# DrawZeroPoint/Structure-Light-Reconstructor

Hardware: AMD Instinct MI355X
Metric: Mpixels/s decode+unwrap+triangulate, 4096x3000 stereo, 1/2/4/8 GPU (higher is better)
Workload: dtype u8 in, f32 phase/XYZ (f64 undistort + Q reprojection)

## Files before the change

structure-light-reconstructor_amd/capi.py:

```python
import ctypes as C
import os

import numpy as np

_HERE = os.path.dirname(os.path.abspath(__file__))
LIB_PATH = os.path.join(_HERE, "libslr_hip.so")

MF_PLANES = 14
MAX_GRAY_BITS = 16
MEM_HOST, MEM_DEVICE = 0, 1
OPT_MF_MATCH_ALGO = 1
OPT_RECT_DECODE_ALGO = 3
OPT_RECT_DMA_SHAPE = 6
OPT_RECT_DMA_DEPTH = 7
OPT_DEBUG_RECT_RESIDENT = 8
OPT_DEBUG_FLAGS = 9
OPT_DEBUG_K4_STOP = 10
OPT_BATCH_STREAMS = 12
OPT_DEBUG_POISON_SCRATCH = 13
OPT_MF_BATCH_GROUP = 15
OPT_MF_BATCH_DECODE_GROUP = 16
OPT_EVAL_MODEL = 14
OPT_HYBRID_ONE_PASS = 11
OPT_PROFILE_STRIDE = 5
# ... 39 lines not shown
    _fields_ = [("W", C.c_int), ("H", C.c_int), ("mf_form", C.c_int), ("dma_shape", C.c_int), ("dma_depth", C.c_int),
                ("dma_tiles", C.c_uint), ("dma_nofit_tiles", C.c_uint), ("quads_by_class", C.c_uint * 3),
                ("waves_by_mode", C.c_uint * 3), ("lds_nofit_tiles", C.c_uint * 2), ("dma_extra_entries", C.c_uint)]


class FuseDesc(C.Structure):
    _fields_ = [("n_frames", C.c_int), ("W", C.c_int), ("H", C.c_int), ("voxel", C.c_double), ("origin", C.c_double * 3),
                ("min_points", C.c_uint32), ("max_voxels", C.c_uint32)]


class FuseStats(C.Structure):
    _fields_ = [("points", C.c_uint64), ("distinct", C.c_uint64), ("table_entries", C.c_uint64), ("atomics", C.c_uint64)]


DEBUG_FUSE_COUNT_ATOMICS = 512

MODE_GRAY, MODE_GE, MODE_MF = 0, 1, 2
ASSIGN_CYCLIC, ASSIGN_BLOCKED = 0, 1


class Calib(C.Structure):
    _fields_ = [("cam", Camera * 2), ("Q", C.c_double * 16), ("T", C.c_float * 12), ("has_T", C.c_int)]


def make_camera(fc, cc, k, R=None, t=None):
    cam = Camera()
    cam.fc[:] = [float(v) for v in fc]
    cam.cc[:] = [float(v) for v in cc]
    kk = list(k) + [0.0] * (5 - len(k))
    cam.k[:] = [float(v) for v in kk]
# ... 724 lines not shown
```

structure-light-reconstructor_amd/csrc/kernels_rectdma.hip:

```cpp
#include "decode_common.hpp"

#include <stdlib.h>

#if !defined(SLR_EXPERIMENTS) && (defined(SLR_DMA_ABL) || defined(SLR_DMA_FORCE_MODE) || defined(SLR_DMA_CLOCKPROBE))
#error "SLR_DMA_ABL / SLR_DMA_FORCE_MODE / SLR_DMA_CLOCKPROBE are experiment switches: build with -DSLR_EXPERIMENTS"
#endif

namespace slr {

constexpr unsigned kDmaInvalid = 0x80000000u;

template <int TW, int TH, int NT>
struct DmaGeom {
    static constexpr int NWAVES = NT / 64;
    static constexpr int PX = TW * TH / NT;
    static constexpr int NQ = PX / 4;
    static constexpr int QPR = TW / 4;
    static constexpr int BR = TH >= 8 ? 8 : TH, BC = 64 / BR;
    static_assert(QPR % BC == 0 && TH % BR == 0, "quad blocks");
    static __device__ __host__ constexpr int quad_row(int g) { return (g / 64) / (QPR / BC) * BR + (g % 64) / BC; }
    static __device__ __host__ constexpr int quad_col(int g) { return ((g / 64) % (QPR / BC) * BC + (g % 64) % BC) * 4; }
    static constexpr int WPR = TW / 64;
    static constexpr int RPP = NWAVES / WPR;
    static constexpr int CMAX = TW / 16 + 2;
// ... 297 lines not shown
}

struct DmaJob {
    const uint8_t *base;
    unsigned pstride;
    unsigned fringe_skip;
    unsigned stack_bytes;
    const int4 *boxes;
    const unsigned *digest;
    unsigned digest_bytes;
    unsigned entries;
    float *phase;
    uint8_t *valid;
};
struct DmaJobs { DmaJob j[kDmaMaxJobs]; };

__device__ __forceinline__ void dma16(unsigned voff, __amdgpu_buffer_rsrc_t rsrc, unsigned lds_dst, unsigned soff)
{
    unsigned keep;
    asm volatile("s_mov_b32 %0, m0\n\ts_mov_b32 m0, %3\n\ts_nop 0\n\tbuffer_load_dwordx4 %1, %2, %4 offen lds\n\ts_mov_b32 m0, %0"
                 : "=&s"(keep) : "v"(voff), "s"(rsrc), "s"(__builtin_amdgcn_readfirstlane(lds_dst)), "s"(__builtin_amdgcn_readfirstlane(soff)) : "memory");
}

template <int N>
__device__ __forceinline__ void wait_vm()
{
    static_assert(N >= 0 && N < 64, "vmcnt is a 6-bit counter");
    asm volatile("s_waitcnt vmcnt(%0)" :: "n"(N) : "memory");
}

// ... 162 lines not shown
        }
    } else {
        DmaRd r[2];
        dma_rd<IMG0, IMG1, RS>(r[0], tap[0].a0);
#pragma unroll
        for (int q = 0; q < PX; q++) {
            if (q + 1 < PX) { dma_rd<IMG0, IMG1, RS>(r[(q + 1) & 1], tap[q + 1].a0); dma_rd_wait<8>(r[q & 1]); }
            else dma_rd_wait<0>(r[q & 1]);
            sd[q] = (int)(dma_blend(r[q & 1], 0, tap[q]) >> 16) - (int)(dma_blend(r[q & 1], 1, tap[q]) >> 16);
        }
    }
}

constexpr int kDmaDigestPhase = 3;
template <int PX, int A, int PLANE_DMAS = 2>
__device__ __host__ constexpr int dma_wait_count(int p)
{
    int n = 0;
    for (int j = 1; j < A; j++) { const int ph = ((p - A + j) % 7 + 7) % 7; n += PLANE_DMAS + (ph == kDmaDigestPhase ? PX / 4 : 0); }
    return n;
}

constexpr int kSubBands = 4;
struct DmaPool {
    int pb;
    int per;
    int T, E;
    int per_x;
    __device__ __host__ static DmaPool of(int T, int E = 0, int x = 0)
    {
        DmaPool p;
        p.pb = (T + 8 * kSubBands - 1) / (8 * kSubBands); p.per = kSubBands * p.pb; p.T = T; p.E = E > T ? E : T;
        p.per_x = 0;
        for (int k = 0; k < kSubBands; k++) {
// ... 99 lines not shown
        if (!has_next) { voff_next = kDmaInvalid; nxt_act = false; }
    }
};

template <int TW, int TH, int NT, int A, bool HASVALID, bool X87 = false>
struct DmaDecode {
    typedef DmaGeom<TW, TH, NT> Gm;
    static constexpr int PX = Gm::PX, PS = Gm::PS, RS = Gm::RS, D = A + 1;
    static constexpr bool SPLIT = 2 * Gm::NCH <= NT;
    static constexpr int PLANE_DMAS = SPLIT ? 1 : 2;
    static constexpr int DIG_OFF = D * 2 * PS, DIG_BYTES = TW * TH * 4;
    static constexpr int WT_OFF = DIG_OFF + DIG_BYTES, WT1_OFF = WT_OFF + 1026 * 4, WT_BYTES = 2 * 1026 * 4;
    static constexpr int TAP_WT = WT_OFF;
    static constexpr int LUT_OFF = WT_OFF + WT_BYTES;
    static constexpr int TKT_OFF = LUT_OFF + (kLutWords + 1) * 4;
    static constexpr int LDS_BYTES = TKT_OFF + 12;
    static_assert(WT_OFF <= 65536 && LDS_BYTES <= 160 * 1024, "DMA destinations are 16-bit LDS addresses (M0)");
    static constexpr int kSentinel = kDmaSentinel;

    const uint8_t *smem;
    const float *lut;
    unsigned lds0, wave_off;
    unsigned pslot_off;
    unsigned plane_g;
    bool plane_wave;
    __amdgpu_buffer_rsrc_t rs_stack, rs_dig, rs_phase, rs_valid;
    unsigned pstride, fringe_skip;
    int W, H, black_thr;
    DmaSched sc;
    DmaTap tap[PX];
    unsigned qbase[PX / 4];
    unsigned oslot[PX / 4];
    unsigned second;
    int mode;
    unsigned ok;
    int pm[PX];
    int dd[PX];
    int Pk[PX];
    float F12[PX];
    float outv[PX];
    unsigned out_ok;
    int out_ty, out_tx;
    bool out_pending;

// ... 34 lines not shown
                dma16(voff, rs_stack, lds0 + (unsigned)((buf * 2 + g) * PS) + pslot_off,
                      (unsigned)dma_phase_plane(p, g) * pstride + (p == 0 ? 0u : fringe_skip));
        }
    }
    __device__ __forceinline__ void issue_digest(unsigned tile, bool live) const
    {
#if defined(SLR_DMA_ABL) && (SLR_DMA_ABL == 8 || SLR_DMA_ABL == 9)
        tile = (tile & 63u) * 94u;
#endif
#pragma unroll
        for (int r = 0; r < PX / 4; r++) {
            const unsigned voff = live ? tile * (unsigned)DIG_BYTES + (threadIdx.x + (unsigned)(NT * r)) * 16u : kDmaInvalid;
            dma16(voff, rs_dig, lds0 + (unsigned)(DIG_OFF + r * NT * 16) + wave_off, 0u);
        }
    }

    static __device__ __forceinline__ float pair_q24(int Pa, int Pb) { return dma_pair_q24(Pa, Pb); }
    static __device__ __forceinline__ float finish_q24(float Fa, float Fb)
    {
        if constexpr (X87) return het_finish_x87(Fa, Fb);
        else return dma_finish_q24(Fa, Fb);
    }

    template <int K0, int P>
    __device__ __forceinline__ void phase(int ty, int tx, unsigned voff_cur)
    {
        static_assert(7 - A > 2 && kDmaDigestPhase > 2 && kDmaDigestPhase < 7, "the next tile is known from phase 2 on");
        if (plane_wave) wait_vm<dma_wait_count<PX, A, PLANE_DMAS>(P)>();
        else if (P == 0) wait_vm<0>();
#if !defined(SLR_DMA_ABL) || SLR_DMA_ABL != 3
        asm volatile("s_barrier" ::: "memory");
#endif
        if (P == 1) sc.draw();
        if constexpr (P == 2) sc.pick_up();
        if (P == kDmaDigestPhase) issue_digest((unsigned)sc.nxt, sc.has_next);
        issue_planes((P + A) % 7, (K0 + P + A) % D, P + A >= 7 ? sc.voff_next : voff_cur);
        if constexpr (P == 0) {
            if (out_pending) flush();
            const unsigned *dg = reinterpret_cast<const unsigned *>(smem + DIG_OFF + threadIdx.x * (PX * 4));
            mode = dma_tap_setup<PX, RS, TAP_WT, WT1_OFF>(smem, lds0, dg, tap, qbase, second, oslot);
            ok = 0;
        }
        constexpr unsigned img0 = (unsigned)(((K0 + P) % D) * 2 * PS), img1 = img0 + PS;
        int sd[PX];
#if defined(SLR_DMA_ABL) && (SLR_DMA_ABL == 2 || SLR_DMA_ABL == 6)
#pragma unroll
        for (int q = 0; q < PX; q++) {
            DmaRd r;
#pragma unroll
            for (int i = 0; i < 8; i++) r.v[i] = tap[q].a0 * (unsigned)(i + 3 + P);
            sd[q] = (int)(dma_blend(r, 0, tap[q]) >> 16) - (int)(dma_blend(r, 1, tap[q]) >> 16);
        }
#elif defined(SLR_DMA_ABL) && SLR_DMA_ABL == 4
#pragma unroll
        for (int q = 0; q < PX; q++) sd[q] = (int)tap[q].a0 + P;
#elif defined(SLR_DMA_ABL) && SLR_DMA_ABL == 5
        DmaRd r[2];
        dma_rd<img0, img1, (unsigned)RS>(r[0], tap[0].a0);
#pragma unroll
        for (int q = 0; q < PX; q++) {
            if (q + 1 < PX) { dma_rd<img0, img1, (unsigned)RS>(r[(q + 1) & 1], tap[q + 1].a0); dma_rd_wait<8>(r[q & 1]); }
            else dma_rd_wait<0>(r[q & 1]);
            sd[q] = (int)(r[q & 1].v[0] ^ r[q & 1].v[1] ^ r[q & 1].v[2] ^ r[q & 1].v[3] ^ r[q & 1].v[4] ^ r[q & 1].v[5] ^ r[q & 1].v[6] ^ r[q & 1].v[7]) & 255;
        }
#else
        __builtin_amdgcn_s_setprio(1);
        if constexpr (P >= 2 && (P & 1) == 0) dma_differences<PX, img1, img0, (unsigned)RS>(mode, tap, qbase, second, sd);
        else dma_differences<PX, img0, img1, (unsigned)RS>(mode, tap, qbase, second, sd);
        __builtin_amdgcn_s_setprio(0);
#endif
        if (P == 1) sc.publish();
        if constexpr (P == 0) {
#pragma unroll
            for (int q = 0; q < PX; q++) {
                if constexpr (HASVALID) ok |= (sd[q] > black_thr ? 0x10001u : 0u) << q;
                else pm[q] = sd[q] > black_thr ? (int)0x80000000 : kSentinel;
            }
        } else if constexpr ((P & 1) != 0) {
#pragma unroll
            for (int q = 0; q < PX; q++) dd[q] = sd[q];
        } else {
#pragma unroll
            for (int q = 0; q < PX; q++) {
                int nz;
                const int Pw = wrapped_nd_q24(sd[q], dd[q], lut, nz);
                if constexpr (HASVALID) { if (nz == 0) ok &= ~(1u << q); }
// ... 4 lines not shown
                    if constexpr (HASVALID) {
                        outv[q] = ((ok >> (q + 16)) & 1u) ? ph : 0.0f;
                    } else {
                        const int m3 = pm[q] > Pw ? pm[q] : Pw;
                        outv[q] = m3 != kSentinel ? ph : kInvalidPhase;
                    }
                }
            }
            if constexpr (P == 6) { out_ok = ok; out_ty = ty; out_tx = tx; out_pending = true; }
        }
    }

    template <int K0, int P>
    __device__ __forceinline__ void idle_phase(unsigned voff_cur)
    {
        if (plane_wave) wait_vm<dma_wait_count<PX, A, PLANE_DMAS>(P)>();
        else if (P == 0) wait_vm<0>();
        asm volatile("s_barrier" ::: "memory");
        if (P == 1) sc.draw();
        if constexpr (P == 2) sc.pick_up();
        if (P == kDmaDigestPhase) issue_digest((unsigned)sc.nxt, sc.has_next);
        issue_planes((P + A) % 7, (K0 + P + A) % D, P + A >= 7 ? sc.voff_next : voff_cur);
        if constexpr (P == 0) { if (out_pending) flush(); out_pending = false; }
        if (P == 1) sc.publish();
    }

    template <int K0>
    __device__ __forceinline__ void tile(int ty, int tx, bool act, unsigned voff_cur)
    {
        if (act) {
            phase<K0, 0>(ty, tx, voff_cur);
            phase<K0, 1>(ty, tx, voff_cur);
            phase<K0, 2>(ty, tx, voff_cur);
            phase<K0, 3>(ty, tx, voff_cur);
            phase<K0, 4>(ty, tx, voff_cur);
            phase<K0, 5>(ty, tx, voff_cur);
            phase<K0, 6>(ty, tx, voff_cur);
        } else {
            idle_phase<K0, 0>(voff_cur);
// ... 8 lines not shown
};

template <int LDS_BYTES, int NT>
constexpr int dma_waves_per_simd()
{
    constexpr int wgs = 160 * 1024 / LDS_BYTES, w = wgs * NT / 256;
    return w > 8 ? 8 : w < 1 ? 1 : w;
}

template <int LDS_BYTES, int NT>
constexpr int mf_dma_waves() { return dma_waves_per_simd<LDS_BYTES, NT>() > 6 ? 6 : dma_waves_per_simd<LDS_BYTES, NT>(); }

template <int TW, int TH, int NT, int A, bool HASVALID, bool X87 = false>
__global__ __launch_bounds__(NT, (HASVALID ? 4 : mf_dma_waves<DmaDecode<TW, TH, NT, A, HASVALID>::LDS_BYTES, NT>())) SLR_TICKET_KERNEL
void mf_rect_decode_dma_kernel(DmaJobs jobs, int njobs, int pitch, int W, int H, int black_thr, const float *__restrict__ lut_g,
                               int tiles_x, int tiles_y, unsigned *__restrict__ sched)
{
    typedef DmaDecode<TW, TH, NT, A, HASVALID, X87> Dec;
    typedef DmaGeom<TW, TH, NT> Gm;
    extern __shared__ __attribute__((aligned(16))) uint8_t smem[];
    Dec d;
    d.smem = smem;
    d.lds0 = __builtin_amdgcn_readfirstlane((unsigned)(uintptr_t)smem);
    if (d.lds0 & 0x1FFFu) __builtin_trap();
#if defined(SLR_DMA_CLOCKPROBE)
    const unsigned long long probe_entry = wall_clock64();
#endif
    float *lut = reinterpret_cast<float *>(smem + Dec::LUT_OFF);
    d.lut = lut;
    for (int i = threadIdx.x; i < kLutWords; i += NT) lut[i] = lut_g[i];
    if constexpr (Dec::WT_BYTES > 0)
    for (unsigned i = threadIdx.x; i < 1025u; i += NT) {
        unsigned w0, w1;
        dma_weights(i, w0, w1);
        *reinterpret_cast<unsigned *>(smem + Dec::WT_OFF + 4u * i) = w0;
        *reinterpret_cast<unsigned *>(smem + Dec::WT1_OFF + 4u * i) = w1;
    }
    __syncthreads();
    if (!HASVALID && threadIdx.x == 0)
        reinterpret_cast<int *>(lut)[kLutP + (9 << 8)] = Dec::kSentinel;
    __syncthreads();
    const unsigned nblk = gridDim.x / (unsigned)njobs;
    const int xcd = (int)(blockIdx.x & 7u), nbx = (int)(nblk >> 3);
    const int ji = (int)((blockIdx.x >> 3) % (unsigned)njobs), lb = (int)((blockIdx.x >> 3) / (unsigned)njobs);
    const int T = tiles_x * tiles_y;
    d.sc.pool = DmaPool::of(T, (int)jobs.j[ji].entries, xcd);
    int cur = d.sc.pool.entry(xcd, lb);
    if (cur < 0) {
        if (threadIdx.x == 0) dma_sched_leave(sched);
        return;
    }

    d.wave_off = __builtin_amdgcn_readfirstlane((threadIdx.x >> 6) * 1024u);
    {
        const unsigned wv = __builtin_amdgcn_readfirstlane(threadIdx.x >> 6);
        constexpr unsigned wpp = (unsigned)Gm::NCH / 64u;
        d.plane_g = Dec::SPLIT ? wv / wpp : 0u;
        d.pslot_off = (Dec::SPLIT ? wv % wpp : wv) * 1024u;
        d.plane_wave = Dec::SPLIT ? wv < 2u * wpp : wv < wpp;
    }
    d.W = W; d.H = H; d.black_thr = black_thr;
    d.sc.pitch = pitch; d.sc.W = W; d.sc.H = H;
    const int chunk = Dec::SPLIT ? (int)threadIdx.x % Gm::NCH : (int)threadIdx.x;
    d.sc.crow = chunk / Gm::CMAX; d.sc.ccol = chunk - d.sc.crow * Gm::CMAX;
    d.sc.chunk_live = Dec::SPLIT || chunk < Gm::NCH;
    d.sc.xcd = xcd; d.sc.first_ticket = nbx;
    d.sc.wave0 = __builtin_amdgcn_readfirstlane(threadIdx.x >> 6) == 0u;
    d.sc.wave_bit = 1u << __builtin_amdgcn_readfirstlane(threadIdx.x >> 6);
    d.sc.tkt_lds = d.lds0 + (unsigned)Dec::TKT_OFF;

#if defined(SLR_DMA_CLOCKPROBE)
    const unsigned long long probe_c0 = clock64(), probe_w0 = wall_clock64();
#endif
    d.pstride = jobs.j[ji].pstride; d.fringe_skip = jobs.j[ji].fringe_skip;
    d.rs_stack = __builtin_amdgcn_make_buffer_rsrc((void *)jobs.j[ji].base, 0, (int)jobs.j[ji].stack_bytes, 0x00020000);
    d.rs_dig = __builtin_amdgcn_make_buffer_rsrc((void *)jobs.j[ji].digest, 0, (int)jobs.j[ji].digest_bytes, 0x00020000);
    d.rs_phase = __builtin_amdgcn_make_buffer_rsrc((void *)jobs.j[ji].phase, 0, (int)((unsigned)W * (unsigned)H * 4u), 0x00020000);
    d.rs_valid = __builtin_amdgcn_make_buffer_rsrc((void *)jobs.j[ji].valid, 0, HASVALID ? (int)((unsigned)W * (unsigned)H) : 0, 0x00020000);
    d.sc.boxes = jobs.j[ji].boxes;
    d.sc.ctr = sched + (ji * 8 + xcd) * kSchedStride;
    d.sc.nxt = 0; d.sc.has_next = false; d.sc.voff_next = kDmaInvalid; d.sc.nxt_ty = d.sc.nxt_tx = 0; d.sc.nxt_act = false;
#if defined(SLR_DMA_CLOCKPROBE)
    int it = 0;
#define SLR_DMA_COUNT(x) ((x)++)
#else
#define SLR_DMA_COUNT(x) ((void)0)
#endif
    int cur_ty, cur_tx;
    bool cur_act;
    unsigned voff_cur = d.sc.box_voff(cur, cur_ty, cur_tx, cur_act);
    d.out_pending = false;
    d.ok = 0;
    d.issue_digest((unsigned)cur, true);
#pragma unroll
    for (int a = 0; a < A; a++) d.issue_planes(a, a % Dec::D, voff_cur);

    for (;;) {
#define SLR_DMA_TILE(K0)                                                                                       \
        {                                                                                                      \
            d.template tile<K0>(cur_ty, cur_tx, cur_act, voff_cur);                                            \
            SLR_DMA_COUNT(it);                                                                                 \
            if (!d.sc.has_next) break;                                                                         \
            cur = d.sc.nxt; voff_cur = d.sc.voff_next;                                                         \
            cur_ty = d.sc.nxt_ty; cur_tx = d.sc.nxt_tx; cur_act = d.sc.nxt_act;                                \
        }
        SLR_DMA_TILE(0)
        SLR_DMA_TILE(7 % Dec::D)
        if constexpr (Dec::D >= 3) SLR_DMA_TILE(14 % Dec::D)
        if constexpr (Dec::D >= 4) SLR_DMA_TILE(21 % Dec::D)
#undef SLR_DMA_TILE
    }
#undef SLR_DMA_COUNT
    if (d.out_pending) d.flush();
    wait_vm<0>();
    if (threadIdx.x == 0) dma_sched_leave(sched);
#if defined(SLR_DMA_CLOCKPROBE)
    if (threadIdx.x == 0) {
        unsigned long long *o = reinterpret_cast<unsigned long long *>(jobs.j[0].phase) + 4 * blockIdx.x;
        unsigned xcc;
// ... 84 lines not shown
    if (bytes >= (1ll << 31) || (long long)W * H * 4 >= (1ll << 31)) return false;
    const char *b = reinterpret_cast<const char *>(tiles);
    j.base = pl.p[0]; j.pstride = (unsigned)st; j.fringe_skip = (unsigned)skip; j.stack_bytes = (unsigned)bytes;
    j.boxes = reinterpret_cast<const int4 *>(b);
    j.digest = reinterpret_cast<const unsigned *>(b + dma_digest_offset(W, H, shape));
    const size_t dg = dma_entry_capacity(W, H, shape) * (size_t)(dma_shape_tw(shape) * dma_shape_th(shape)) * 4;
    if (dg >= (1ull << 31)) return false;
    j.digest_bytes = (unsigned)dg;
    j.entries = (unsigned)dma_tile_count(W, H, shape);
    j.phase = phase; j.valid = valid;
    return true;
}

template <int TW, int TH, int NT, int A, bool HV, bool X87 = false>
static hipError_t launch_dma_variant(const DmaJobs &j, int njobs, int pitch, int W, int H, int black_thr, const float *lut, unsigned *sched,
                                     hipStream_t s)
{
    typedef DmaDecode<TW, TH, NT, A, HV, X87> Dec;
    auto kern = mf_rect_decode_dma_kernel<TW, TH, NT, A, HV, X87>;
    static DevSlots resident;
    int dev = 0;
    (void)hipGetDevice(&dev);
    int res = resident.get(dev);
    if (!res) {
        hipError_t e0 = hipFuncSetAttribute((const void *)kern, hipFuncAttributeMaxDynamicSharedMemorySize, Dec::LDS_BYTES);
        if (e0 != hipSuccess) return e0;
        int per_cu = 0, cus = 0;
        if (hipOccupancyMaxActiveBlocksPerMultiprocessor(&per_cu, kern, NT, Dec::LDS_BYTES) != hipSuccess || per_cu < 1) per_cu = 1;
        if (hipDeviceGetAttribute(&cus, hipDeviceAttributeMultiprocessorCount, dev) != hipSuccess || cus < 1) cus = 256;
        res = per_cu * cus;
        resident.put(dev, res);
    }
    const int tiles_x = (W + TW - 1) / TW, tiles_y = (H + TH - 1) / TH;
    const int T = tiles_x * tiles_y, per = DmaPool::of(T).per;
    const int r = (tl_debug.rect_resident > 0 ? tl_debug.rect_resident : res) / njobs;
    int nbx = r / 8 < per ? r / 8 : per;
    if (nbx < 1) nbx = 1;
    hipError_t e = hipMemsetAsync(sched, 0, kSchedBytes, s);
    if (e != hipSuccess) return e;
    SLR_LAUNCH(kern, dim3(8u * (unsigned)nbx * (unsigned)njobs), dim3(NT), Dec::LDS_BYTES, s, j, njobs, pitch, W, H, black_thr, lut,
               tiles_x, tiles_y, sched);
    return hipGetLastError();
}

#define SLR_DMA_DEPTH2(TW, TH, NT) 2
hipError_t launch_mf_rect_decode_dma(const MfPlanes *pl, int n, int pitch, int W, int H, int black_thr, const float *lut,
                                     float *const *phase, uint8_t *const *valid, const void *const *tiles, int shape, int depth,
                                     unsigned *sched, const DmaFixup *fix, bool *done, hipStream_t s, const int *fix_slot)
{
    *done = false;
    if (shape < 0 || shape >= kDmaShapes || !sched || n < 1 || n > kDmaMaxJobs) return hipSuccess;
    auto slot = [&](int c) { return fix_slot ? fix_slot[c] : c; };
    for (int c = 0; c < n; c++)
        if (fix && fix->nofit[slot(c)] > 0 && (!fix->map_xy[slot(c)] || !fix->map_frac[slot(c)])) return hipSuccess;
    DmaJobs j;
    for (int c = 0; c < n; c++) {
        if (!dma_job(pl[c], pitch, W, H, phase[c], valid[c], tiles[c], shape, j.j[c])) return hipSuccess;
        if (fix) j.j[c].entries += fix->extras[slot(c)];
    }
    for (int c = n; c < kDmaMaxJobs; c++) j.j[c] = j.j[0];
    const bool hv = valid[0] != nullptr;
    for (int c = 1; c < n; c++) if ((valid[c] != nullptr) != hv) return hipSuccess;
    *done = true;
    hipError_t e = hipSuccess;
    const bool x87 = tl_debug.eval_x87;
#define SLR_DMA_X(TW, TH, NT)                                                                                          \
    e = x87        ? (hv ? launch_dma_variant<TW, TH, NT, SLR_DMA_DEPTH2(TW, TH, NT), true, true>(j, n, pitch, W, H, black_thr, lut, sched, s)     \
                         : launch_dma_variant<TW, TH, NT, SLR_DMA_DEPTH2(TW, TH, NT), false, true>(j, n, pitch, W, H, black_thr, lut, sched, s))   \
      : depth >= 2 ? (hv ? launch_dma_variant<TW, TH, NT, SLR_DMA_DEPTH2(TW, TH, NT), true>(j, n, pitch, W, H, black_thr, lut, sched, s)     \
                         : launch_dma_variant<TW, TH, NT, SLR_DMA_DEPTH2(TW, TH, NT), false>(j, n, pitch, W, H, black_thr, lut, sched, s))   \
                   : (hv ? launch_dma_variant<TW, TH, NT, 1, true>(j, n, pitch, W, H, black_thr, lut, sched, s)              \
                         : launch_dma_variant<TW, TH, NT, 1, false>(j, n, pitch, W, H, black_thr, lut, sched, s))
    SLR_DMA_SHAPE_SWITCH(shape, SLR_DMA_X)
#undef SLR_DMA_X
    for (int c = 0; c < n && e == hipSuccess; c++) {
        if (!fix || fix->nofit[slot(c)] == 0) continue;
        const unsigned cnt = fix->nofit[slot(c)];
        const int tiles_x = (W + dma_shape_tw(shape) - 1) / dma_shape_tw(shape);
#define SLR_DMA_X(TW, TH, NT)                                                                                          \
        if (x87) hipLaunchKernelGGL((mf_rect_fixup_kernel<TW, TH, true>), dim3(cnt * (unsigned)(TW * TH / 256) < 16384u ? cnt * (unsigned)(TW * TH / 256) : 16384u), dim3(256), 0, s, pl[c], pitch, W, H, black_thr, \
                           lut, fix->map_xy[slot(c)], fix->map_frac[slot(c)], dma_nofit_list(tiles[c], W, H, shape), cnt, tiles_x, phase[c], valid[c]); \
        else hipLaunchKernelGGL((mf_rect_fixup_kernel<TW, TH>), dim3(cnt * (unsigned)(TW * TH / 256) < 16384u ? cnt * (unsigned)(TW * TH / 256) : 16384u), dim3(256), 0, s, pl[c], pitch, W, H, black_thr, \
                           lut, fix->map_xy[slot(c)], fix->map_frac[slot(c)], dma_nofit_list(tiles[c], W, H, shape), cnt, tiles_x, phase[c], valid[c])
        SLR_DMA_SHAPE_SWITCH(shape, SLR_DMA_X)
#undef SLR_DMA_X
        e = hipGetLastError();
    }
// ... 554 lines not shown
```

structure-light-reconstructor_amd/csrc/slr_capi.hip:

```cpp
#include "slr_device.hpp"

#include <math.h>
#include <stdio.h>
#include <string.h>

#include <new>
#include <string>
#include <vector>

using namespace slr;

namespace {

const char *kKernelNames[K_COUNT] = {
    "slr_remap_u8", "slr_mf_decode", "slr_mf_rectify_decode", "slr_gray_decode", "slr_gray_rectify_decode",
    "slr_mf_match_triangulate", "slr_ge_match_triangulate", "slr_ray_count", "slr_ray_scan", "slr_ray_scatter",
    "slr_ray_triangulate",
    "slr_pc_from_grid", "slr_pc_get", "slr_undistort_table", "slr_ray_table", "slr_mf_rectify_decode_pair", "slr_mfn_decode",
    "slr_gray_rectify_decode_pair", "slr_hybrid_rectify_decode_pair", "slr_mfn_rectify_decode",
    "slr_fuse_clear", "slr_fuse_insert", "slr_fuse_total", "slr_fuse_flag", "slr_fuse_scan", "slr_fuse_emit"};

enum Slot {
    S_STAGE0 = 0,
    S_PHASE_L = 16, S_VALID_L, S_PHASE_R, S_VALID_R,
// ... 1071 lines not shown
        for (int cam = 0; cam < 2; cam++) {
            if (sets) mp[2 * f + cam] = sets[2 * f + cam];
            else {
                const uint8_t *base = stack + (size_t)f * 2 * SLR_MF_PLANES * plane + (size_t)cam * SLR_MF_PLANES * plane;
                for (int i = 0; i < SLR_MF_PLANES; i++) mp[2 * f + cam].p[i] = base + plane * i;
            }
            ph[2 * f + cam] = (cam ? phR : phL) + (size_t)f * n;
            vd[2 * f + cam] = nullptr;
            tl[2 * f + cam] = c->d_dma_tiles[cam];
            slot[2 * f + cam] = cam;
        }
    const DmaFixup fix = dma_fixup_of(c, 0, 1);
    ProfScope ps(c, K_MF_RECT_DECODE_PAIR, true);
    ps.r.units = g;
    SLR_HIP(c, launch_mf_rect_decode_dma(mp, 2 * g, pitch, W, H, black_thr, c->d_lut, ph, vd, tl, c->opt_dma_shape, c->opt_dma_depth,
                                         c->d_sched, &fix, grouped, c->stream, slot));
    return SLR_OK;
}

static int reconstruct_mf_dev(slr_ctx *c, const uint8_t *const *pL, const uint8_t *const *pR, int pitch, int W, int H,
                              int black_thr, int rectify, float *xyz, uint8_t *has)
{
    const size_t n = (size_t)W * H;
    void *phL, *phR;
    SLR_TRY(get_scratch(c, S_PHASE_L, n * 4, &phL));
    SLR_TRY(get_scratch(c, S_PHASE_R, n * 4, &phR));
    SLR_TRY(decode_pair_dev(c, pL, pR, pitch, W, H, black_thr, rectify, (float *)phL, nullptr, (float *)phR, nullptr));
    return core_mf_match(c, (const float *)phL, nullptr, (const float *)phR, nullptr, W, H, xyz, has, nullptr);
}

static int mf_batch_group_of(const slr_ctx *c, int W, int rectify, int H = 0, const float *xyz = nullptr, const uint8_t *has = nullptr)
// ... 907 lines not shown
            if (value < 0 || value > 6) return fail(c, SLR_ERR_INVALID_ARG, "SLR_OPT_RECT_DMA_SHAPE must be 0..6");
            if (value == 2 || value >= 4) return fail(c, SLR_ERR_UNSUPPORTED, "SLR_OPT_RECT_DMA_SHAPE = 2, 4, 5, 6 are retired forms");
            if (value != c->opt_dma_shape) {
                c->opt_dma_shape = value;
                SLR_TRY(use_device(c));
                for (int cam = 0; cam < 2; cam++)
                    if (c->d_map_xy[cam]) SLR_TRY(build_dma_tiles(c, cam));
                SLR_HIP(c, hipStreamSynchronize(c->stream));
            }
            return SLR_OK;
        case SLR_OPT_DEBUG_RECT_RESIDENT:
            if (value < 0) return fail(c, SLR_ERR_INVALID_ARG, "SLR_OPT_DEBUG_RECT_RESIDENT must be >= 0");
            c->debug.rect_resident = value;
            return SLR_OK;
        case SLR_OPT_DEBUG_FLAGS:
            if (value < 0 || value > 1023) return fail(c, SLR_ERR_INVALID_ARG, "SLR_OPT_DEBUG_FLAGS must be 0..1023");
            c->debug.fuse_count_atomics = (value & 512) != 0;
            c->debug.mfn_nt512 = (value & 128) != 0;
            c->debug.mfn_ring4 = (value & 256) != 0;
            c->debug.no_tiled_map = (value & 1) != 0;
            c->debug.no_buffer_form = (value & 2) != 0;
            c->debug.no_ge_lean = (value & 4) != 0;
            c->debug.no_decode_count = (value & 8) != 0;
            c->debug.gray_small_tiles = (value & 16) != 0;
            if (c->debug.no_quad_sort != ((value & 32) != 0) || c->debug.no_promote != ((value & 64) != 0)) {
                c->debug.no_quad_sort = (value & 32) != 0;
                c->debug.no_promote = (value & 64) != 0;
                SLR_TRY(use_device(c));
                for (int cam = 0; cam < 2; cam++)
                    if (c->d_map_xy[cam] && c->d_dma_tiles[cam]) SLR_TRY(build_dma_tiles(c, cam));
                SLR_HIP(c, hipStreamSynchronize(c->stream));
            }
// ... 128 lines not shown
```

structure-light-reconstructor_amd/csrc/slr_device.hpp:

```cpp
#pragma once

#include <hip/hip_runtime.h>
#include <hip/hip_ext.h>
#include <stdint.h>

#include <atomic>

#include "slr.h"

namespace slr {

constexpr float kPI = 3.1416f;
constexpr float kTwoPI = 2 * kPI;
constexpr float kThreeHalfPI = 3 * kPI / 2;
constexpr float kHalfPI = kPI / 2;
constexpr int kDecodeLutWords = 512 + 10 * 256 + 1;

struct DevSlots {
    std::atomic<int> v[64];
    int get(int dev) const { return (unsigned)dev < 64u ? v[dev].load(std::memory_order_relaxed) : 0; }
    void put(int dev, int x) { if ((unsigned)dev < 64u) v[dev].store(x, std::memory_order_relaxed); }
};

struct MfPlanes { const uint8_t *p[SLR_MF_PLANES]; };
// ... 24 lines not shown

struct DebugKnobs {
    int rect_resident = 0;
    bool no_tiled_map = false;
    bool no_buffer_form = false;
    bool no_ge_lean = false;
    bool no_decode_count = false;
    bool no_quad_sort = false;
    bool no_promote = false;
    bool gray_small_tiles = false;
    bool mfn_nt512 = false;
    bool mfn_ring4 = false;
    int k4_stop = 0;
    bool poison_scratch = false;
    bool fuse_count_atomics = false;
    bool eval_x87 = false;
};
extern thread_local DebugKnobs tl_debug;
#define SLR_LAUNCH(kernel, grid, block, lds, stream, ...)                                                            \
    do {                                                                                                             \
        if (::slr::tl_prof_start) {                                                                                  \
            hipExtLaunchKernelGGL(kernel, grid, block, (uint32_t)(lds), stream, ::slr::tl_prof_start, ::slr::tl_prof_stop, 0, \
                                  __VA_ARGS__);                                                                      \
            ::slr::tl_prof_start = nullptr;                                                                          \
        } else {                                                                                                     \
            hipLaunchKernelGGL(kernel, grid, block, lds, stream, __VA_ARGS__);                                       \
        }                                                                                                            \
    } while (0)

hipError_t launch_remap_u8(const uint8_t *src, int src_pitch, uint8_t *dst, int dst_pitch, int W, int H,
// ... 23 lines not shown
size_t     dma_tile_count_of(int W, int H, int shape);
unsigned   dma_extra_entries_capacity(int W, int H, int shape);
hipError_t launch_dma_tiles(const int16_t *map_xy, const uint16_t *map_frac, int W, int H, void *buf, int shape,
                            bool promote ,
                            bool sort_quads ,
                            unsigned *nofit_host, hipStream_t s);
struct DmaFixup {
    const int16_t *map_xy[2];
    const uint16_t *map_frac[2];
    unsigned nofit[2];
    unsigned extras[2];
};
hipError_t launch_mf_rect_decode_dma(const MfPlanes *pl, int n, int pitch, int W, int H, int black_thr, const float *lut,
                                     float *const *phase, uint8_t *const *valid, const void *const *tiles, int shape, int depth,
                                     unsigned *sched ,
                                     const DmaFixup *fix, bool *done, hipStream_t s, const int *fix_slot = nullptr);
constexpr int kDmaMaxJobs = 16;
size_t     dma_sched_bytes();

hipError_t launch_gray_rect_decode_dma(const GrayPlanes *pl, int n, int ncol, int nrow, int pitch, int W, int H, int black_thr,
                                       int white_thr, int scan_w, int scan_h, int32_t *const *code_x, int32_t *const *code_y,
                                       uint8_t *const *valid, const void *const *tiles, int shape, int depth , unsigned *sched, const DmaFixup *fix,
                                       bool *done, hipStream_t s, const int *fix_slot = nullptr);
hipError_t launch_hybrid_rect_decode_dma(const GrayPlanes *pl, int n, int ncol, int pitch, int W, int H, int black_thr, int white_thr,
                                         int scan_w, const float *lut, int32_t *const *code_x, float *const *phase,
                                         const void *const *tiles, int shape, unsigned *sched, const DmaFixup *fix, bool *done,
                                         hipStream_t s);
hipError_t launch_gray_decode(const GrayPlanes &pl, int n_col_bits, int n_row_bits, int pitch, int W, int H,
                              int black_thr, int white_thr, int scan_w, int scan_h,
                              int32_t *code_x, int32_t *code_y, uint8_t *valid,
                              const int16_t *map_xy, const uint16_t *map_frac, const void *tile_boxes, int rect_algo,
                              hipStream_t s);
// ... 127 lines not shown
```

Baseline: 64880.

## Decode several frames per tile visit reusing tap setup and schedule

```diff
diff --git a/profiles/decode_visits_ab.py b/profiles/decode_visits_ab.py
--- /dev/null
+++ b/profiles/decode_visits_ab.py
@@ -0,0 +1,84 @@
+import argparse
+import json
+import os
+import sys
+import time
+
+ROOT = os.path.dirname(os.path.dirname(os.path.abspath(__file__)))
+sys.path.insert(0, ROOT)
+
+
+def main():
+    ap = argparse.ArgumentParser()
+    ap.add_argument("--rounds", type=int, default=4)
+    ap.add_argument("--batches", type=int, default=20)
+    ap.add_argument("--warmup", type=int, default=4)
+    ap.add_argument("--lib", default=None, help="another build of libslr_hip.so (experiments)")
+    ap.add_argument("--legs", default="0,1024", help="SLR_OPT_DEBUG_FLAGS of the legs of a round (alternating order)")
+    ap.add_argument("--x87", type=int, default=0)
+    ap.add_argument("--width", type=int, default=4096)
+    ap.add_argument("--height", type=int, default=3000)
+    args = ap.parse_args()
+    import importlib
+    import torch
+    capi = importlib.import_module("structure-light-reconstructor_amd.capi")
+    if args.lib:
+        capi.LIB_PATH = os.path.abspath(args.lib)
+    slr = importlib.import_module("structure-light-reconstructor_amd")
+    synth = importlib.import_module("structure-light-reconstructor_amd.synth")
+    W, H, F, BLACK = args.width, args.height, 8, 40
+    dev = torch.device("cuda", 0)
+    ctx = slr.Context(0)
+    if args.x87:
+        ctx.set_option(capi.OPT_EVAL_MODEL, 1)
+    rig = synth.make_verged_rig(W, H, 0.2, -0.15)
+    ctx.set_calibration(rig["calib"])
+    synth.install_verged_maps(ctx, rig, W, H)
+    stack = torch.stack([synth.render_mf_stack(W, H, seed=1000 + f, noise=2, device=dev) for f in range(F)])
+    xyz = torch.empty((F, H, W, 3), dtype=torch.float32, device=dev)
+    has = torch.empty((F, H, W), dtype=torch.uint8, device=dev)
+    torch.cuda.synchronize()
+    ctx.set_option(capi.OPT_PROFILE_STRIDE, 1)
+    legs = [int(v) for v in args.legs.split(",")]
+    res = {f: [] for f in legs}
+    sums = {}
+    for r in range(args.rounds):
+        for flags in (legs if r % 2 == 0 else legs[::-1]):
+            ctx.set_option(capi.OPT_DEBUG_FLAGS, flags)
+            for _ in range(args.warmup):
+                ctx.reconstruct_mf_batch(stack, BLACK, True, xyz=xyz, has=has)
+            ctx.synchronize()
+            ctx.profile_enable(True)
+            ctx.profile_reset()
+            t0 = time.perf_counter()
+            for _ in range(args.batches):
+                ctx.reconstruct_mf_batch(stack, BLACK, True, xyz=xyz, has=has)
+            ctx.synchronize()
+            wall = time.perf_counter() - t0
+            pr = ctx.profile()
+            ctx.profile_enable(False)
+            leg = {"round": r, "debug_flags": flags, "wall_ms_per_frame": round(wall / (args.batches * F) * 1e3, 4)}
+            for kn, short in (("slr_mf_rectify_decode_pair", "decode_us_per_frame"), ("slr_mf_match_triangulate", "match_us_per_frame")):
+                if kn in pr and pr[kn][1]:
+                    leg[short] = round(pr[kn][0] / pr[kn][1] * 1e3, 2)
+            sums.setdefault(flags, set()).add(tuple(int(v) for v in ctx.cloud_checksums(xyz, has)))
+            res[flags].append(leg)
+            print(json.dumps(leg), flush=True)
+    ctx.set_option(capi.OPT_DEBUG_FLAGS, 0)
+    summ = {"lib": args.lib or "in-tree", "x87": args.x87, "rounds": args.rounds, "batches_per_leg": args.batches,
+            "same_clouds": all(sums[f] == sums[legs[0]] for f in legs) and len(sums[legs[0]]) == 1}
+    for flags, entries in res.items():
+        for k in ("decode_us_per_frame", "match_us_per_frame", "wall_ms_per_frame"):
+            v = sorted(e[k] for e in entries if k in e)
+            if v:
+                summ["flags_%d_%s" % (flags, k)] = {"min": v[0], "median": v[len(v) // 2], "max": v[-1]}
+    a, b = summ.get("flags_%d_decode_us_per_frame" % legs[0]), summ.get("flags_%d_decode_us_per_frame" % legs[-1])
+    if a and b and len(legs) == 2:
+        summ["decode_gain_median"] = round(1.0 - a["median"] / b["median"], 4)
+    summ["checksums"] = ["%016x" % (v & 0xFFFFFFFFFFFFFFFF) for v in sorted(sums[legs[0]])[0]]
+    print(json.dumps(summ), flush=True)
+    ctx.close()
+
+
+if __name__ == "__main__":
+    main()
diff --git a/structure-light-reconstructor_amd/capi.py b/structure-light-reconstructor_amd/capi.py
--- a/structure-light-reconstructor_amd/capi.py
+++ b/structure-light-reconstructor_amd/capi.py
@@ -77,6 +77,7 @@
 
 
 DEBUG_FUSE_COUNT_ATOMICS = 512
+DEBUG_ONE_FRAME_VISITS = 1024
 
 MODE_GRAY, MODE_GE, MODE_MF = 0, 1, 2
 ASSIGN_CYCLIC, ASSIGN_BLOCKED = 0, 1
diff --git a/structure-light-reconstructor_amd/csrc/kernels_rectdma.hip b/structure-light-reconstructor_amd/csrc/kernels_rectdma.hip
--- a/structure-light-reconstructor_amd/csrc/kernels_rectdma.hip
+++ b/structure-light-reconstructor_amd/csrc/kernels_rectdma.hip
@@ -335,6 +335,7 @@
     uint8_t *valid;
 };
 struct DmaJobs { DmaJob j[kDmaMaxJobs]; };
+constexpr int kDmaMaxVisit = kDmaMaxJobs / 2;
 
 __device__ __forceinline__ void dma16(unsigned voff, __amdgpu_buffer_rsrc_t rsrc, unsigned lds_dst, unsigned soff)
 {
@@ -527,10 +528,10 @@
 
 constexpr int kDmaDigestPhase = 3;
 template <int PX, int A, int PLANE_DMAS = 2>
-__device__ __host__ constexpr int dma_wait_count(int p)
+__device__ __host__ constexpr int dma_wait_count(int p, bool digest = true)
 {
     int n = 0;
-    for (int j = 1; j < A; j++) { const int ph = ((p - A + j) % 7 + 7) % 7; n += PLANE_DMAS + (ph == kDmaDigestPhase ? PX / 4 : 0); }
+    for (int j = 1; j < A; j++) { const int ph = ((p - A + j) % 7 + 7) % 7; n += PLANE_DMAS + (digest && ph == kDmaDigestPhase ? PX / 4 : 0); }
     return n;
 }
 
@@ -660,7 +661,8 @@
     static constexpr int TAP_WT = WT_OFF;
     static constexpr int LUT_OFF = WT_OFF + WT_BYTES;
     static constexpr int TKT_OFF = LUT_OFF + (kLutWords + 1) * 4;
-    static constexpr int LDS_BYTES = TKT_OFF + 12;
+    static constexpr int FRM_OFF = (TKT_OFF + 12 + 15) & ~15;
+    static constexpr int LDS_BYTES = FRM_OFF + 16 * kDmaMaxVisit;
     static_assert(WT_OFF <= 65536 && LDS_BYTES <= 160 * 1024, "DMA destinations are 16-bit LDS addresses (M0)");
     static constexpr int kSentinel = kDmaSentinel;
 
@@ -674,6 +676,8 @@
     unsigned pstride, fringe_skip;
     int W, H, black_thr;
     DmaSched sc;
+    int fk, fn;
+    unsigned stack_bytes;
     DmaTap tap[PX];
     unsigned qbase[PX / 4];
     unsigned oslot[PX / 4];
@@ -738,6 +742,16 @@
             dma16(voff, rs_dig, lds0 + (unsigned)(DIG_OFF + r * NT * 16) + wave_off, 0u);
         }
     }
+    __device__ __forceinline__ bool last_frame() const { return fk + 1 >= fn; }
+    __device__ __forceinline__ __amdgpu_buffer_rsrc_t frame_rsrc(int k, int which) const
+    {
+        unsigned long long v;
+        asm volatile("ds_read_b64 %0, %1\n\ts_waitcnt lgkmcnt(0)" : "=v"(v) : "v"(lds0 + (unsigned)(FRM_OFF + 16 * k + 8 * which)) : "memory");
+        const unsigned long long p = (unsigned long long)(unsigned)__builtin_amdgcn_readfirstlane((unsigned)v) |
+                                     (unsigned long long)(unsigned)__builtin_amdgcn_readfirstlane((unsigned)(v >> 32)) << 32;
+        return __builtin_amdgcn_make_buffer_rsrc((void *)(uintptr_t)p, 0, which ? (int)((unsigned)W * (unsigned)H * 4u) : (int)stack_bytes,
+                                                 0x00020000);
+    }
 
     static __device__ __forceinline__ float pair_q24(int Pa, int Pb) { return dma_pair_q24(Pa, Pb); }
     static __device__ __forceinline__ float finish_q24(float Fa, float Fb)
@@ -746,23 +760,43 @@
         else return dma_finish_q24(Fa, Fb);
     }
 
+    template <int P>
+    __device__ __forceinline__ void unit_wait(bool last) const
+    {
+        constexpr int n = dma_wait_count<PX, A, PLANE_DMAS>(P), n0 = dma_wait_count<PX, A, PLANE_DMAS>(P, false);
+        if (plane_wave) {
+            if constexpr (n == n0) wait_vm<n>();
+            else if (last) wait_vm<n>();
+            else wait_vm<n0>();
+        } else if (P == 0) wait_vm<0>();
+    }
+    template <int K0, int P>
+    __device__ __forceinline__ void unit_schedule(bool last, unsigned voff_cur)
+    {
+        if (P == 1 && last) sc.draw();
+        if constexpr (P == 2) { if (last) sc.pick_up(); }
+        if (P == kDmaDigestPhase && last) issue_digest((unsigned)sc.nxt, sc.has_next);
+        if (P == 7 - A && fn > 1) rs_stack = frame_rsrc(last ? 0 : fk + 1, 0);
+        issue_planes((P + A) % 7, (K0 + P + A) % D, P + A >= 7 && last ? sc.voff_next : voff_cur);
+    }
+
     template <int K0, int P>
     __device__ __forceinline__ void phase(int ty, int tx, unsigned voff_cur)
     {
         static_assert(7 - A > 2 && kDmaDigestPhase > 2 && kDmaDigestPhase < 7, "the next tile is known from phase 2 on");
-        if (plane_wave) wait_vm<dma_wait_count<PX, A, PLANE_DMAS>(P)>();
-        else if (P == 0) wait_vm<0>();
+        const bool last = last_frame();
+        unit_wait<P>(last);
 #if !defined(SLR_DMA_ABL) || SLR_DMA_ABL != 3
         asm volatile("s_barrier" ::: "memory");
 #endif
-        if (P == 1) sc.draw();
-        if constexpr (P == 2) sc.pick_up();
-        if (P == kDmaDigestPhase) issue_digest((unsigned)sc.nxt, sc.has_next);
-        issue_planes((P + A) % 7, (K0 + P + A) % D, P + A >= 7 ? sc.voff_next : voff_cur);
+        unit_schedule<K0, P>(last, voff_cur);
         if constexpr (P == 0) {
             if (out_pending) flush();
-            const unsigned *dg = reinterpret_cast<const unsigned *>(smem + DIG_OFF + threadIdx.x * (PX * 4));
-            mode = dma_tap_setup<PX, RS, TAP_WT, WT1_OFF>(smem, lds0, dg, tap, qbase, second, oslot);
+            if (fn > 1) rs_phase = frame_rsrc(fk, 1);
+            if (fk == 0) {
+                const unsigned *dg = reinterpret_cast<const unsigned *>(smem + DIG_OFF + threadIdx.x * (PX * 4));
+                mode = dma_tap_setup<PX, RS, TAP_WT, WT1_OFF>(smem, lds0, dg, tap, qbase, second, oslot);
+            }
             ok = 0;
         }
         constexpr unsigned img0 = (unsigned)(((K0 + P) % D) * 2 * PS), img1 = img0 + PS;
@@ -793,7 +827,7 @@
         else dma_differences<PX, img0, img1, (unsigned)RS>(mode, tap, qbase, second, sd);
         __builtin_amdgcn_s_setprio(0);
 #endif
-        if (P == 1) sc.publish();
+        if (P == 1 && last) sc.publish();
         if constexpr (P == 0) {
 #pragma unroll
             for (int q = 0; q < PX; q++) {
@@ -828,15 +862,12 @@
     template <int K0, int P>
     __device__ __forceinline__ void idle_phase(unsigned voff_cur)
     {
-        if (plane_wave) wait_vm<dma_wait_count<PX, A, PLANE_DMAS>(P)>();
-        else if (P == 0) wait_vm<0>();
+        const bool last = last_frame();
+        unit_wait<P>(last);
         asm volatile("s_barrier" ::: "memory");
-        if (P == 1) sc.draw();
-        if constexpr (P == 2) sc.pick_up();
-        if (P == kDmaDigestPhase) issue_digest((unsigned)sc.nxt, sc.has_next);
-        issue_planes((P + A) % 7, (K0 + P + A) % D, P + A >= 7 ? sc.voff_next : voff_cur);
+        unit_schedule<K0, P>(last, voff_cur);
         if constexpr (P == 0) { if (out_pending) flush(); out_pending = false; }
-        if (P == 1) sc.publish();
+        if (P == 1 && last) sc.publish();
     }
 
     template <int K0>
@@ -875,7 +906,7 @@
 template <int TW, int TH, int NT, int A, bool HASVALID, bool X87 = false>
 __global__ __launch_bounds__(NT, (HASVALID ? 4 : mf_dma_waves<DmaDecode<TW, TH, NT, A, HASVALID>::LDS_BYTES, NT>())) SLR_TICKET_KERNEL
 void mf_rect_decode_dma_kernel(DmaJobs jobs, int njobs, int pitch, int W, int H, int black_thr, const float *__restrict__ lut_g,
-                               int tiles_x, int tiles_y, unsigned *__restrict__ sched)
+                               int tiles_x, int tiles_y, unsigned *__restrict__ sched, int nsets, int nframes)
 {
     typedef DmaDecode<TW, TH, NT, A, HASVALID, X87> Dec;
     typedef DmaGeom<TW, TH, NT> Gm;
@@ -898,12 +929,25 @@
         *reinterpret_cast<unsigned *>(smem + Dec::WT1_OFF + 4u * i) = w1;
     }
     __syncthreads();
+    const unsigned nblk = gridDim.x / (unsigned)njobs;
+    const int xcd = (int)(blockIdx.x & 7u), nbx = (int)(nblk >> 3);
+    const int vi = (int)((blockIdx.x >> 3) % (unsigned)njobs), lb = (int)((blockIdx.x >> 3) / (unsigned)njobs);
+    int ji = vi;
+    d.fk = 0; d.fn = 1;
+    if (nsets > 0) {
+        const int s = vi >> 1, f0 = s * nframes / nsets, f1 = (s + 1) * nframes / nsets;
+        ji = 2 * f0 + (vi & 1);
+        d.fn = f1 - f0;
+        if (threadIdx.x == 0)
+            for (int k = 0; k < d.fn; k++) {
+                unsigned long long *t = reinterpret_cast<unsigned long long *>(smem + Dec::FRM_OFF + 16 * k);
+                t[0] = (unsigned long long)(uintptr_t)jobs.j[ji + 2 * k].base;
+                t[1] = (unsigned long long)(uintptr_t)jobs.j[ji + 2 * k].phase;
+            }
+    }
     if (!HASVALID && threadIdx.x == 0)
         reinterpret_cast<int *>(lut)[kLutP + (9 << 8)] = Dec::kSentinel;
     __syncthreads();
-    const unsigned nblk = gridDim.x / (unsigned)njobs;
-    const int xcd = (int)(blockIdx.x & 7u), nbx = (int)(nblk >> 3);
-    const int ji = (int)((blockIdx.x >> 3) % (unsigned)njobs), lb = (int)((blockIdx.x >> 3) / (unsigned)njobs);
     const int T = tiles_x * tiles_y;
     d.sc.pool = DmaPool::of(T, (int)jobs.j[ji].entries, xcd);
     int cur = d.sc.pool.entry(xcd, lb);
@@ -934,12 +978,13 @@
     const unsigned long long probe_c0 = clock64(), probe_w0 = wall_clock64();
 #endif
     d.pstride = jobs.j[ji].pstride; d.fringe_skip = jobs.j[ji].fringe_skip;
+    d.stack_bytes = jobs.j[ji].stack_bytes;
     d.rs_stack = __builtin_amdgcn_make_buffer_rsrc((void *)jobs.j[ji].base, 0, (int)jobs.j[ji].stack_bytes, 0x00020000);
     d.rs_dig = __builtin_amdgcn_make_buffer_rsrc((void *)jobs.j[ji].digest, 0, (int)jobs.j[ji].digest_bytes, 0x00020000);
     d.rs_phase = __builtin_amdgcn_make_buffer_rsrc((void *)jobs.j[ji].phase, 0, (int)((unsigned)W * (unsigned)H * 4u), 0x00020000);
     d.rs_valid = __builtin_amdgcn_make_buffer_rsrc((void *)jobs.j[ji].valid, 0, HASVALID ? (int)((unsigned)W * (unsigned)H) : 0, 0x00020000);
     d.sc.boxes = jobs.j[ji].boxes;
-    d.sc.ctr = sched + (ji * 8 + xcd) * kSchedStride;
+    d.sc.ctr = sched + (vi * 8 + xcd) * kSchedStride;
     d.sc.nxt = 0; d.sc.has_next = false; d.sc.voff_next = kDmaInvalid; d.sc.nxt_ty = d.sc.nxt_tx = 0; d.sc.nxt_act = false;
 #if defined(SLR_DMA_CLOCKPROBE)
     int it = 0;
@@ -961,9 +1006,13 @@
         {                                                                                                      \
             d.template tile<K0>(cur_ty, cur_tx, cur_act, voff_cur);                                            \
             SLR_DMA_COUNT(it);                                                                                 \
-            if (!d.sc.has_next) break;                                                                         \
-            cur = d.sc.nxt; voff_cur = d.sc.voff_next;                                                         \
-            cur_ty = d.sc.nxt_ty; cur_tx = d.sc.nxt_tx; cur_act = d.sc.nxt_act;                                \
+            if (!d.last_frame()) d.fk++;                         \
+            else {                                                                                             \
+                d.fk = 0;                                                                                      \
+                if (!d.sc.has_next) break;                                                                     \
+                cur = d.sc.nxt; voff_cur = d.sc.voff_next;                                                     \
+                cur_ty = d.sc.nxt_ty; cur_tx = d.sc.nxt_tx; cur_act = d.sc.nxt_act;                            \
+            }                                                                                                  \
         }
         SLR_DMA_TILE(0)
         SLR_DMA_TILE(7 % Dec::D)
@@ -1078,8 +1127,10 @@
 
 template <int TW, int TH, int NT, int A, bool HV, bool X87 = false>
 static hipError_t launch_dma_variant(const DmaJobs &j, int njobs, int pitch, int W, int H, int black_thr, const float *lut, unsigned *sched,
-                                     hipStream_t s)
-{
+                                     hipStream_t s, int nsets)
+{
+    const int nframes = njobs / 2;
+    if (nsets > 0) njobs = 2 * nsets;
     typedef DmaDecode<TW, TH, NT, A, HV, X87> Dec;
     auto kern = mf_rect_decode_dma_kernel<TW, TH, NT, A, HV, X87>;
     static DevSlots resident;
@@ -1103,14 +1154,14 @@
     hipError_t e = hipMemsetAsync(sched, 0, kSchedBytes, s);
     if (e != hipSuccess) return e;
     SLR_LAUNCH(kern, dim3(8u * (unsigned)nbx * (unsigned)njobs), dim3(NT), Dec::LDS_BYTES, s, j, njobs, pitch, W, H, black_thr, lut,
-               tiles_x, tiles_y, sched);
+               tiles_x, tiles_y, sched, nsets, nframes);
     return hipGetLastError();
 }
 
 #define SLR_DMA_DEPTH2(TW, TH, NT) 2
 hipError_t launch_mf_rect_decode_dma(const MfPlanes *pl, int n, int pitch, int W, int H, int black_thr, const float *lut,
                                      float *const *phase, uint8_t *const *valid, const void *const *tiles, int shape, int depth,
-                                     unsigned *sched, const DmaFixup *fix, bool *done, hipStream_t s, const int *fix_slot)
+                                     unsigned *sched, const DmaFixup *fix, bool *done, hipStream_t s, const int *fix_slot, int visit_frames)
 {
     *done = false;
     if (shape < 0 || shape >= kDmaShapes || !sched || n < 1 || n > kDmaMaxJobs) return hipSuccess;
@@ -1125,16 +1176,27 @@
     for (int c = n; c < kDmaMaxJobs; c++) j.j[c] = j.j[0];
     const bool hv = valid[0] != nullptr;
     for (int c = 1; c < n; c++) if ((valid[c] != nullptr) != hv) return hipSuccess;
+    int nsets = 0;
+    if (n > 2 && n % 2 == 0 && visit_frames > 1 && !hv) {
+        bool same = true;
+        for (int c = 2; c < n; c++) {
+            const DmaJob &a = j.j[c], &b = j.j[c & 1];
+            same = same && a.pstride == b.pstride && a.fringe_skip == b.fringe_skip && a.stack_bytes == b.stack_bytes && a.boxes == b.boxes &&
+                   a.digest == b.digest && a.digest_bytes == b.digest_bytes && a.entries == b.entries;
+        }
+        const int g = n / 2, f = visit_frames < kDmaMaxVisit ? visit_frames : kDmaMaxVisit;
+        if (same) nsets = (g + f - 1) / f;
+    }
     *done = true;
     hipError_t e = hipSuccess;
     const bool x87 = tl_debug.eval_x87;
 #define SLR_DMA_X(TW, TH, NT)                                                                                          \
-    e = x87        ? (hv ? launch_dma_variant<TW, TH, NT, SLR_DMA_DEPTH2(TW, TH, NT), true, true>(j, n, pitch, W, H, black_thr, lut, sched, s)     \
-                         : launch_dma_variant<TW, TH, NT, SLR_DMA_DEPTH2(TW, TH, NT), false, true>(j, n, pitch, W, H, black_thr, lut, sched, s))   \
-      : depth >= 2 ? (hv ? launch_dma_variant<TW, TH, NT, SLR_DMA_DEPTH2(TW, TH, NT), true>(j, n, pitch, W, H, black_thr, lut, sched, s)     \
-                         : launch_dma_variant<TW, TH, NT, SLR_DMA_DEPTH2(TW, TH, NT), false>(j, n, pitch, W, H, black_thr, lut, sched, s))   \
-                   : (hv ? launch_dma_variant<TW, TH, NT, 1, true>(j, n, pitch, W, H, black_thr, lut, sched, s)              \
-                         : launch_dma_variant<TW, TH, NT, 1, false>(j, n, pitch, W, H, black_thr, lut, sched, s))
+    e = x87        ? (hv ? launch_dma_variant<TW, TH, NT, SLR_DMA_DEPTH2(TW, TH, NT), true, true>(j, n, pitch, W, H, black_thr, lut, sched, s, nsets)     \
+                         : launch_dma_variant<TW, TH, NT, SLR_DMA_DEPTH2(TW, TH, NT), false, true>(j, n, pitch, W, H, black_thr, lut, sched, s, nsets))   \
+      : depth >= 2 ? (hv ? launch_dma_variant<TW, TH, NT, SLR_DMA_DEPTH2(TW, TH, NT), true>(j, n, pitch, W, H, black_thr, lut, sched, s, nsets)     \
+                         : launch_dma_variant<TW, TH, NT, SLR_DMA_DEPTH2(TW, TH, NT), false>(j, n, pitch, W, H, black_thr, lut, sched, s, nsets))   \
+                   : (hv ? launch_dma_variant<TW, TH, NT, 1, true>(j, n, pitch, W, H, black_thr, lut, sched, s, nsets)              \
+                         : launch_dma_variant<TW, TH, NT, 1, false>(j, n, pitch, W, H, black_thr, lut, sched, s, nsets))
     SLR_DMA_SHAPE_SWITCH(shape, SLR_DMA_X)
 #undef SLR_DMA_X
     for (int c = 0; c < n && e == hipSuccess; c++) {
diff --git a/structure-light-reconstructor_amd/csrc/slr_capi.hip b/structure-light-reconstructor_amd/csrc/slr_capi.hip
--- a/structure-light-reconstructor_amd/csrc/slr_capi.hip
+++ b/structure-light-reconstructor_amd/csrc/slr_capi.hip
@@ -1109,7 +1109,7 @@
     ProfScope ps(c, K_MF_RECT_DECODE_PAIR, true);
     ps.r.units = g;
     SLR_HIP(c, launch_mf_rect_decode_dma(mp, 2 * g, pitch, W, H, black_thr, c->d_lut, ph, vd, tl, c->opt_dma_shape, c->opt_dma_depth,
-                                         c->d_sched, &fix, grouped, c->stream, slot));
+                                         c->d_sched, &fix, grouped, c->stream, slot, c->debug.one_frame_visits ? 1 : kDmaVisitFrames));
     return SLR_OK;
 }
 
@@ -2047,8 +2047,9 @@
             c->debug.rect_resident = value;
             return SLR_OK;
         case SLR_OPT_DEBUG_FLAGS:
-            if (value < 0 || value > 1023) return fail(c, SLR_ERR_INVALID_ARG, "SLR_OPT_DEBUG_FLAGS must be 0..1023");
+            if (value < 0 || value > 2047) return fail(c, SLR_ERR_INVALID_ARG, "SLR_OPT_DEBUG_FLAGS must be 0..2047");
             c->debug.fuse_count_atomics = (value & 512) != 0;
+            c->debug.one_frame_visits = (value & 1024) != 0;
             c->debug.mfn_nt512 = (value & 128) != 0;
             c->debug.mfn_ring4 = (value & 256) != 0;
             c->debug.no_tiled_map = (value & 1) != 0;
diff --git a/structure-light-reconstructor_amd/csrc/slr_device.hpp b/structure-light-reconstructor_amd/csrc/slr_device.hpp
--- a/structure-light-reconstructor_amd/csrc/slr_device.hpp
+++ b/structure-light-reconstructor_amd/csrc/slr_device.hpp
@@ -62,6 +62,7 @@
     int k4_stop = 0;
     bool poison_scratch = false;
     bool fuse_count_atomics = false;
+    bool one_frame_visits = false;
     bool eval_x87 = false;
 };
 extern thread_local DebugKnobs tl_debug;
@@ -115,8 +116,10 @@
 hipError_t launch_mf_rect_decode_dma(const MfPlanes *pl, int n, int pitch, int W, int H, int black_thr, const float *lut,
                                      float *const *phase, uint8_t *const *valid, const void *const *tiles, int shape, int depth,
                                      unsigned *sched ,
-                                     const DmaFixup *fix, bool *done, hipStream_t s, const int *fix_slot = nullptr);
+                                     const DmaFixup *fix, bool *done, hipStream_t s, const int *fix_slot = nullptr,
+                                     int visit_frames = 1 );
 constexpr int kDmaMaxJobs = 16;
+constexpr int kDmaVisitFrames = 8;
 size_t     dma_sched_bytes();
 
 hipError_t launch_gray_rect_decode_dma(const GrayPlanes *pl, int n, int ncol, int nrow, int pitch, int W, int H, int black_thr,
```

Measured after the change: 66000, median of 6. 1.02x the previous value.
